# CompVis/zigma

Hardware: AMD Instinct MI355X
Metric: denoiser-forward latents/sec (BxL tokens/s), ZigMa d=640 L=32^2 (higher is better)
Workload: dtype bf16; 1 GPU; readme_text_b64: ZigMa(in_ch=3,img=32,E=640,depth=18,zigzagN8,has_text 77x768), B=64/GPU, bf16, one forward per step; global_batch=64, seq_len=1024, parallelism=batch-sharded x1

## Files before the change

zigma_amd/csrc/cross_attn.hip:

```cpp
#include "zigma_common.h"

namespace zigma {

typedef __bf16 bf16x8 __attribute__((ext_vector_type(8)));
typedef float f32x4 __attribute__((ext_vector_type(4)));

constexpr int kXaD = 64;
constexpr int kXaWaves = 4, kXaTok = 16;
constexpr int kXaKPitch = (kXaD + 8) * 2;


typedef float xa_f32x2 __attribute__((ext_vector_type(2)));
typedef __bf16 xa_bf16x2 __attribute__((ext_vector_type(2)));
__device__ __forceinline__ uint32_t pack_bf16(float lo, float hi) {
    return __builtin_bit_cast(uint32_t, __builtin_convertvector(xa_f32x2{lo, hi}, xa_bf16x2));
}

template <int NKB, bool MASK_ALL>
__global__ __launch_bounds__(64 * kXaWaves) void cross_attn_kernel(const zigma_xattn_params_t p, const int kXaTiles) {
    constexpr int KP = 16 * NKB;
    constexpr int KS = (KP + 31) / 32, KP2 = 32 * KS;
    constexpr int VPitch = (KP2 + 8) * 2;
    constexpr int OPitch = kXaKPitch;
    static_assert(VPitch >= OPitch, "the O tile reuses the P tile");
    __shared__ __attribute__((aligned(16))) unsigned char s_k[KP * kXaKPitch];
    __shared__ __attribute__((aligned(16))) unsigned char s_vt[kXaD * VPitch];
    __shared__ __attribute__((aligned(16))) unsigned char s_p[kXaWaves][kXaTok * VPitch];

    const int tid = threadIdx.x, lane = tid & 63;
    const int wave = __builtin_amdgcn_readfirstlane(tid >> 6);
    const int h = blockIdx.y, b = blockIdx.z, L = p.seqlen, NC = p.n_ctx;
    const int i16 = lane & 15, g = lane >> 4;
    const uint16_t *qb = reinterpret_cast<const uint16_t *>(p.q) + b * p.q_batch_stride + h * kXaD;
    const uint16_t *kb = reinterpret_cast<const uint16_t *>(p.k) + b * p.k_batch_stride + h * kXaD;
    const uint16_t *vb = reinterpret_cast<const uint16_t *>(p.v) + b * p.v_batch_stride + h * kXaD;
    uint16_t *ob = reinterpret_cast<uint16_t *>(p.out) + b * p.o_batch_stride + h * kXaD;

    for (int piece = tid; piece < KP * 8; piece += 64 * kXaWaves) {
        const int row = piece >> 3, pc = piece & 7;
        uint4 kv = make_uint4(0, 0, 0, 0);
        if (row < NC) kv = *reinterpret_cast<const uint4 *>(kb + row * p.k_row_stride + pc * 8);
        *reinterpret_cast<uint4 *>(s_k + row * kXaKPitch + pc * 16) = kv;
    }
    for (int unit = tid; unit < (KP2 / 8) * (kXaD / 2); unit += 64 * kXaWaves) {
        const int kg = unit / (kXaD / 2), dp = unit % (kXaD / 2);
        uint32_t w[8];
#pragma unroll
        for (int e = 0; e < 8; ++e) {
            const int key = kg * 8 + e;
            w[e] = key < NC ? *reinterpret_cast<const uint32_t *>(vb + key * p.v_row_stride + dp * 2) : 0u;
        }
        uint4 lo, hi;
        lo.x = (w[0] & 0xffffu) | (w[1] << 16); lo.y = (w[2] & 0xffffu) | (w[3] << 16);
        lo.z = (w[4] & 0xffffu) | (w[5] << 16); lo.w = (w[6] & 0xffffu) | (w[7] << 16);
        hi.x = (w[0] >> 16) | (w[1] & 0xffff0000u); hi.y = (w[2] >> 16) | (w[3] & 0xffff0000u);
        hi.z = (w[4] >> 16) | (w[5] & 0xffff0000u); hi.w = (w[6] >> 16) | (w[7] & 0xffff0000u);
        *reinterpret_cast<uint4 *>(s_vt + (2 * dp) * VPitch + kg * 16) = lo;
        *reinterpret_cast<uint4 *>(s_vt + (2 * dp + 1) * VPitch + kg * 16) = hi;
    }
    __syncthreads();

    const float sc = p.scale * kLog2e;
    unsigned char *pt = s_p[wave];
    const int tile0 = blockIdx.x * kXaTiles * kXaWaves + wave;
    auto load_q = [&](int t0, bf16x8 (&qa)[2]) {
        int tq = t0 + i16;
        tq = tq < L ? tq : L - 1;
        const uint16_t *qrow = qb + static_cast<int64_t>(tq) * p.q_row_stride;
#pragma unroll
        for (int ks = 0; ks < 2; ++ks) qa[ks] = __builtin_bit_cast(bf16x8, *reinterpret_cast<const uint4 *>(qrow + ks * 32 + g * 8));
    };
    bf16x8 qn[2];
    if (tile0 * kXaTok < L) load_q(tile0 * kXaTok, qn);
#pragma unroll 1
    for (int it = 0; it < kXaTiles; ++it) {
        const int t0 = (tile0 + it * kXaWaves) * kXaTok;
        if (t0 >= L) break;
        const bf16x8 qa[2] = {qn[0], qn[1]};
        if (it + 1 < kXaTiles && t0 + kXaWaves * kXaTok < L) load_q(t0 + kXaWaves * kXaTok, qn);
        f32x4 s[NKB];
#pragma unroll
        for (int ks = 0; ks < 2; ++ks) {
#pragma unroll
            for (int nb = 0; nb < NKB; ++nb) {
                const bf16x8 kf = __builtin_bit_cast(bf16x8, *reinterpret_cast<const uint4 *>(s_k + (nb * 16 + i16) * kXaKPitch + ks * 64 + g * 16));
                s[nb] = ks == 0 ? __builtin_amdgcn_mfma_f32_16x16x32_bf16(kf, qa[ks], f32x4{0.f, 0.f, 0.f, 0.f}, 0, 0, 0)
                                : __builtin_amdgcn_mfma_f32_16x16x32_bf16(kf, qa[ks], s[nb], 0, 0, 0);
            }
        }
        float m = -INFINITY;
#pragma unroll
        for (int nb = 0; nb < NKB; ++nb) {
#pragma unroll
            for (int r = 0; r < 4; ++r) {
                if (MASK_ALL || nb == NKB - 1) s[nb][r] = (nb * 16 + 4 * g + r < NC) ? s[nb][r] : -INFINITY;
                m = fmaxf(m, s[nb][r]);
            }
        }
        m = fmaxf(m, __shfl_xor(m, 16, 64));
        m = fmaxf(m, __shfl_xor(m, 32, 64));
        const float msc = -m * sc;
        float sum = 0.f;
#pragma unroll
        for (int nb = 0; nb < NKB; ++nb) {
            float e[4];
#pragma unroll
            for (int r = 0; r < 4; ++r) { e[r] = fast_exp2(__builtin_fmaf(s[nb][r], sc, msc)); sum += e[r]; }
            *reinterpret_cast<uint2 *>(pt + i16 * VPitch + (nb * 16 + 4 * g) * 2) = make_uint2(pack_bf16(e[0], e[1]), pack_bf16(e[2], e[3]));
        }
        if (KP2 > KP) *reinterpret_cast<uint2 *>(pt + i16 * VPitch + (KP + 4 * g) * 2) = make_uint2(0u, 0u);
        sum += __shfl_xor(sum, 16, 64);
        sum += __shfl_xor(sum, 32, 64);
        __builtin_amdgcn_fence(__ATOMIC_RELEASE, "wavefront");
        __builtin_amdgcn_wave_barrier();
        __builtin_amdgcn_fence(__ATOMIC_ACQUIRE, "wavefront");
        f32x4 o[4];
#pragma unroll
        for (int ks = 0; ks < KS; ++ks) {
            const bf16x8 pf = __builtin_bit_cast(bf16x8, *reinterpret_cast<const uint4 *>(pt + i16 * VPitch + ks * 64 + g * 16));
#pragma unroll
            for (int db = 0; db < 4; ++db) {
                const bf16x8 vf = __builtin_bit_cast(bf16x8, *reinterpret_cast<const uint4 *>(s_vt + (db * 16 + i16) * VPitch + ks * 64 + g * 16));
                o[db] = ks == 0 ? __builtin_amdgcn_mfma_f32_16x16x32_bf16(vf, pf, f32x4{0.f, 0.f, 0.f, 0.f}, 0, 0, 0)
                                : __builtin_amdgcn_mfma_f32_16x16x32_bf16(vf, pf, o[db], 0, 0, 0);
            }
        }
        __builtin_amdgcn_fence(__ATOMIC_RELEASE, "wavefront");
        __builtin_amdgcn_wave_barrier();
        const float inv = fast_rcp(sum);
#pragma unroll
        for (int db = 0; db < 4; ++db)
            *reinterpret_cast<uint2 *>(pt + i16 * OPitch + (db * 16 + 4 * g) * 2) =
                make_uint2(pack_bf16(o[db][0] * inv, o[db][1] * inv), pack_bf16(o[db][2] * inv, o[db][3] * inv));
        __builtin_amdgcn_fence(__ATOMIC_RELEASE, "wavefront");
        __builtin_amdgcn_wave_barrier();
        __builtin_amdgcn_fence(__ATOMIC_ACQUIRE, "wavefront");
#pragma unroll
        for (int q = 0; q < 2; ++q) {
            const int idx = lane + 64 * q, tok = idx >> 3, pc = idx & 7;
            if (t0 + tok < L)
                *reinterpret_cast<uint4 *>(ob + static_cast<int64_t>(t0 + tok) * p.o_row_stride + pc * 8) =
                    *reinterpret_cast<const uint4 *>(pt + tok * OPitch + pc * 16);
        }
        __builtin_amdgcn_fence(__ATOMIC_RELEASE, "wavefront");
        __builtin_amdgcn_wave_barrier();
    }
}

}

using namespace zigma;

extern "C" int zigma_cross_attn_fwd(const zigma_xattn_params_t *pp, void *stream_) {
    if (!pp) return ZIGMA_ERR_NULL;
    (void)hipGetLastError();
    const zigma_xattn_params_t &p = *pp;
    if (p.batch < 0 || p.seqlen < 0 || p.heads < 1 || p.n_ctx < 1) return ZIGMA_ERR_SHAPE;
    if (p.flags != 0) return ZIGMA_ERR_UNSUPPORTED;
    if (!(p.scale > 0.f) || !(p.scale < 3.0e38f)) return ZIGMA_ERR_UNSUPPORTED;
    if (p.batch == 0 || p.seqlen == 0) return ZIGMA_OK;
    if (!p.q || !p.k || !p.v || !p.out) return ZIGMA_ERR_NULL;
    if (p.dtype != ZIGMA_BF16) return ZIGMA_ERR_DTYPE;
    if (p.head_dim != kXaD || p.n_ctx > 128 || p.batch > 65535 || p.heads > 65535) return ZIGMA_ERR_SHAPE;
    auto mis = [](const void *q, int64_t rs, int64_t bs) { return reinterpret_cast<uintptr_t>(q) % 16 != 0 || rs % 8 != 0 || bs % 8 != 0; };
    if (mis(p.q, p.q_row_stride, p.q_batch_stride) || mis(p.k, p.k_row_stride, p.k_batch_stride) ||
        mis(p.v, p.v_row_stride, p.v_batch_stride) || mis(p.out, p.o_row_stride, p.o_batch_stride))
        return ZIGMA_ERR_STRIDE;
    const int tiles = p.seqlen >= 512 ? 8 : 4;
    const int tok_per_wg = kXaTok * kXaWaves * tiles;
    dim3 grid((p.seqlen + tok_per_wg - 1) / tok_per_wg, p.heads, p.batch), block(64 * kXaWaves);
    hipStream_t stream = static_cast<hipStream_t>(stream_);
    if (p.n_ctx <= 80) {
        if (p.n_ctx > 64) hipLaunchKernelGGL((cross_attn_kernel<5, false>), grid, block, 0, stream, p, tiles);
        else hipLaunchKernelGGL((cross_attn_kernel<5, true>), grid, block, 0, stream, p, tiles);
    } else {
        if (p.n_ctx > 112) hipLaunchKernelGGL((cross_attn_kernel<8, false>), grid, block, 0, stream, p, tiles);
        else hipLaunchKernelGGL((cross_attn_kernel<8, true>), grid, block, 0, stream, p, tiles);
    }
    set_last_kernel("cross_attn_mfma");
    return check_launch();
}
```

Measured before the change: 3.855 million tokens/s.

## Prefetch K/V into registers, ring-buffer Q loads, use 8 waves for long sequences

The cross-attention kernel now issues all global K and V loads into registers before any shared-memory stores, so the loads overlap instead of serialising load/store. Q tiles are prefetched through a configurable ring of register slots, and the refill is placed after the QK MFMAs, fenced by sched barriers. For seqlen >= 1024 the launch uses 8 waves per workgroup instead of 4, and waves_per_eu hints are added. Bounds branches become clamped loads and masks. The cost is higher register pressure and fewer workgroups along the sequence axis.

Measured after the change: 3.859 million tokens/s, median of 5. No clear change (+0.1%).

```diff
diff --git a/zigma_amd/csrc/cross_attn.hip b/zigma_amd/csrc/cross_attn.hip
--- a/zigma_amd/csrc/cross_attn.hip
+++ b/zigma_amd/csrc/cross_attn.hip
@@ -6,18 +6,29 @@
 typedef float f32x4 __attribute__((ext_vector_type(4)));
 
 constexpr int kXaD = 64;
-constexpr int kXaWaves = 4, kXaTok = 16;
+constexpr int kXaTok = 16;
+#ifndef ZIGMA_XA_WAVES8_MIN_L
+#define ZIGMA_XA_WAVES8_MIN_L 1024
+#endif
 constexpr int kXaKPitch = (kXaD + 8) * 2;
+#ifndef ZIGMA_XA_RING
+#define ZIGMA_XA_RING 1
+#endif
+#ifndef ZIGMA_XA_TILES
+#define ZIGMA_XA_TILES 8
+#endif
+constexpr int kXaRing = ZIGMA_XA_RING;
 
 
 typedef float xa_f32x2 __attribute__((ext_vector_type(2)));
 typedef __bf16 xa_bf16x2 __attribute__((ext_vector_type(2)));
+typedef uint32_t xa_u32x4 __attribute__((ext_vector_type(4)));
 __device__ __forceinline__ uint32_t pack_bf16(float lo, float hi) {
     return __builtin_bit_cast(uint32_t, __builtin_convertvector(xa_f32x2{lo, hi}, xa_bf16x2));
 }
 
-template <int NKB, bool MASK_ALL>
-__global__ __launch_bounds__(64 * kXaWaves) void cross_attn_kernel(const zigma_xattn_params_t p, const int kXaTiles) {
+template <int NKB, bool MASK_ALL, int kXaWaves>
+__global__ __launch_bounds__(64 * kXaWaves) __attribute__((amdgpu_waves_per_eu(NKB == 5 ? 4 : 3))) void cross_attn_kernel(const zigma_xattn_params_t p, const int kXaTiles) {
     constexpr int KP = 16 * NKB;
     constexpr int KS = (KP + 31) / 32, KP2 = 32 * KS;
     constexpr int VPitch = (KP2 + 8) * 2;
@@ -36,20 +47,66 @@
     const uint16_t *vb = reinterpret_cast<const uint16_t *>(p.v) + b * p.v_batch_stride + h * kXaD;
     uint16_t *ob = reinterpret_cast<uint16_t *>(p.out) + b * p.o_batch_stride + h * kXaD;
 
-    for (int piece = tid; piece < KP * 8; piece += 64 * kXaWaves) {
+    const int tile0 = blockIdx.x * kXaTiles * kXaWaves + wave;
+    const int rem = L - tile0 * kXaTok;
+    const int nt_all = (rem + kXaWaves * kXaTok - 1) / (kXaWaves * kXaTok);
+    const int nt = rem <= 0 ? 0 : (nt_all < kXaTiles ? nt_all : kXaTiles);
+    auto load_q = [&](int t0, xa_u32x4 (&qa)[2]) {
+        int tq = t0 + i16;
+        tq = tq < L ? tq : L - 1;
+        const uint16_t *qrow = qb + static_cast<int64_t>(tq) * p.q_row_stride;
+#pragma unroll
+        for (int ks = 0; ks < 2; ++ks) qa[ks] = *reinterpret_cast<const xa_u32x4 *>(qrow + ks * 32 + g * 8);
+    };
+    xa_u32x4 qr[kXaRing][2];
+#pragma unroll
+    for (int r = 0; r < kXaRing; ++r)
+        load_q(r < nt ? (tile0 + r * kXaWaves) * kXaTok : L, qr[r]);
+
+    constexpr int NT = 64 * kXaWaves, KPieces = KP * 8, VUnits = (KP2 / 8) * (kXaD / 2);
+    constexpr int KI = (KPieces + NT - 1) / NT, VI = (VUnits + NT - 1) / NT;
+    xa_u32x4 kreg[KI];
+    uint32_t vreg[VI][8];
+#pragma unroll
+    for (int i = 0; i < KI; ++i) {
+        int piece = tid + i * NT;
+        piece = piece < KPieces ? piece : KPieces - 1;
+        int row = piece >> 3;
+        row = row < NC ? row : NC - 1;
+        kreg[i] = *reinterpret_cast<const xa_u32x4 *>(kb + row * p.k_row_stride + (piece & 7) * 8);
+    }
+#pragma unroll
+    for (int i = 0; i < VI; ++i) {
+        int unit = tid + i * NT;
+        unit = unit < VUnits ? unit : VUnits - 1;
+        const int kg = unit / (kXaD / 2), dp = unit % (kXaD / 2);
+#pragma unroll
+        for (int e = 0; e < 8; ++e) {
+            int key = kg * 8 + e;
+            key = key < NC ? key : NC - 1;
+#ifdef ZIGMA_XA_PROBE_NO_V
+            vreg[i][e] = 0u;
+#else
+            vreg[i][e] = *reinterpret_cast<const uint32_t *>(vb + key * p.v_row_stride + dp * 2);
+#endif
+        }
+    }
+#pragma unroll
+    for (int i = 0; i < KI; ++i) {
+        int piece = tid + i * NT;
+        piece = piece < KPieces ? piece : KPieces - 1;
         const int row = piece >> 3, pc = piece & 7;
-        uint4 kv = make_uint4(0, 0, 0, 0);
-        if (row < NC) kv = *reinterpret_cast<const uint4 *>(kb + row * p.k_row_stride + pc * 8);
-        *reinterpret_cast<uint4 *>(s_k + row * kXaKPitch + pc * 16) = kv;
-    }
-    for (int unit = tid; unit < (KP2 / 8) * (kXaD / 2); unit += 64 * kXaWaves) {
+        const uint32_t keep = row < NC ? ~0u : 0u;
+        *reinterpret_cast<xa_u32x4 *>(s_k + row * kXaKPitch + pc * 16) = kreg[i] & keep;
+    }
+#pragma unroll
+    for (int i = 0; i < VI; ++i) {
+        int unit = tid + i * NT;
+        unit = unit < VUnits ? unit : VUnits - 1;
         const int kg = unit / (kXaD / 2), dp = unit % (kXaD / 2);
         uint32_t w[8];
 #pragma unroll
-        for (int e = 0; e < 8; ++e) {
-            const int key = kg * 8 + e;
-            w[e] = key < NC ? *reinterpret_cast<const uint32_t *>(vb + key * p.v_row_stride + dp * 2) : 0u;
-        }
+        for (int e = 0; e < 8; ++e) w[e] = kg * 8 + e < NC ? vreg[i][e] : 0u;
         uint4 lo, hi;
         lo.x = (w[0] & 0xffffu) | (w[1] << 16); lo.y = (w[2] & 0xffffu) | (w[3] << 16);
         lo.z = (w[4] & 0xffffu) | (w[5] << 16); lo.w = (w[6] & 0xffffu) | (w[7] << 16);
@@ -58,26 +115,14 @@
         *reinterpret_cast<uint4 *>(s_vt + (2 * dp) * VPitch + kg * 16) = lo;
         *reinterpret_cast<uint4 *>(s_vt + (2 * dp + 1) * VPitch + kg * 16) = hi;
     }
+    __builtin_amdgcn_s_waitcnt(0x0F70);
     __syncthreads();
 
     const float sc = p.scale * kLog2e;
     unsigned char *pt = s_p[wave];
-    const int tile0 = blockIdx.x * kXaTiles * kXaWaves + wave;
-    auto load_q = [&](int t0, bf16x8 (&qa)[2]) {
-        int tq = t0 + i16;
-        tq = tq < L ? tq : L - 1;
-        const uint16_t *qrow = qb + static_cast<int64_t>(tq) * p.q_row_stride;
-#pragma unroll
-        for (int ks = 0; ks < 2; ++ks) qa[ks] = __builtin_bit_cast(bf16x8, *reinterpret_cast<const uint4 *>(qrow + ks * 32 + g * 8));
-    };
-    bf16x8 qn[2];
-    if (tile0 * kXaTok < L) load_q(tile0 * kXaTok, qn);
-#pragma unroll 1
-    for (int it = 0; it < kXaTiles; ++it) {
+    auto do_tile = [&](const int it, xa_u32x4 (&slot)[2], const bool refill) __attribute__((always_inline)) {
         const int t0 = (tile0 + it * kXaWaves) * kXaTok;
-        if (t0 >= L) break;
-        const bf16x8 qa[2] = {qn[0], qn[1]};
-        if (it + 1 < kXaTiles && t0 + kXaWaves * kXaTok < L) load_q(t0 + kXaWaves * kXaTok, qn);
+        const bf16x8 qa[2] = {__builtin_bit_cast(bf16x8, slot[0]), __builtin_bit_cast(bf16x8, slot[1])};
         f32x4 s[NKB];
 #pragma unroll
         for (int ks = 0; ks < 2; ++ks) {
@@ -88,6 +133,11 @@
                                 : __builtin_amdgcn_mfma_f32_16x16x32_bf16(kf, qa[ks], s[nb], 0, 0, 0);
             }
         }
+        if (refill) {
+            __builtin_amdgcn_sched_barrier(0);
+            load_q(it + kXaRing < nt ? t0 + kXaRing * kXaWaves * kXaTok : L, slot);
+            __builtin_amdgcn_sched_barrier(0);
+        }
         float m = -INFINITY;
 #pragma unroll
         for (int nb = 0; nb < NKB; ++nb) {
@@ -137,13 +187,25 @@
         __builtin_amdgcn_fence(__ATOMIC_ACQUIRE, "wavefront");
 #pragma unroll
         for (int q = 0; q < 2; ++q) {
-            const int idx = lane + 64 * q, tok = idx >> 3, pc = idx & 7;
-            if (t0 + tok < L)
-                *reinterpret_cast<uint4 *>(ob + static_cast<int64_t>(t0 + tok) * p.o_row_stride + pc * 8) =
-                    *reinterpret_cast<const uint4 *>(pt + tok * OPitch + pc * 16);
-        }
-        __builtin_amdgcn_fence(__ATOMIC_RELEASE, "wavefront");
-        __builtin_amdgcn_wave_barrier();
+            const int idx = lane + 64 * q, pc = idx & 7;
+            int tok = idx >> 3;
+            tok = t0 + tok < L ? tok : L - 1 - t0;
+            *reinterpret_cast<uint4 *>(ob + static_cast<int64_t>(t0 + tok) * p.o_row_stride + pc * 8) =
+                *reinterpret_cast<const uint4 *>(pt + tok * OPitch + pc * 16);
+        }
+        __builtin_amdgcn_fence(__ATOMIC_RELEASE, "wavefront");
+        __builtin_amdgcn_wave_barrier();
+    };
+    int itb = 0;
+#pragma unroll 1
+    for (; itb + kXaRing <= nt; itb += kXaRing) {
+#pragma unroll
+        for (int r = 0; r < kXaRing; ++r) do_tile(itb + r, qr[r], true);
+    }
+#pragma unroll
+    for (int r = 0; r < kXaRing - 1; ++r) {
+        if (itb + r >= nt) break;
+        do_tile(itb + r, qr[r], false);
     }
 }
 
@@ -166,17 +228,20 @@
     if (mis(p.q, p.q_row_stride, p.q_batch_stride) || mis(p.k, p.k_row_stride, p.k_batch_stride) ||
         mis(p.v, p.v_row_stride, p.v_batch_stride) || mis(p.out, p.o_row_stride, p.o_batch_stride))
         return ZIGMA_ERR_STRIDE;
-    const int tiles = p.seqlen >= 512 ? 8 : 4;
-    const int tok_per_wg = kXaTok * kXaWaves * tiles;
-    dim3 grid((p.seqlen + tok_per_wg - 1) / tok_per_wg, p.heads, p.batch), block(64 * kXaWaves);
+    const int tiles = p.seqlen >= 512 ? ZIGMA_XA_TILES : 4;
+    const int waves = p.seqlen >= ZIGMA_XA_WAVES8_MIN_L ? 8 : 4;
+    const int tok_per_wg = kXaTok * waves * tiles;
+    dim3 grid((p.seqlen + tok_per_wg - 1) / tok_per_wg, p.heads, p.batch), block(64 * waves);
     hipStream_t stream = static_cast<hipStream_t>(stream_);
+#define ZIGMA_XA(NKB_, MASK_) \
+    if (waves == 8) hipLaunchKernelGGL((cross_attn_kernel<NKB_, MASK_, 8>), grid, block, 0, stream, p, tiles); \
+    else hipLaunchKernelGGL((cross_attn_kernel<NKB_, MASK_, 4>), grid, block, 0, stream, p, tiles);
     if (p.n_ctx <= 80) {
-        if (p.n_ctx > 64) hipLaunchKernelGGL((cross_attn_kernel<5, false>), grid, block, 0, stream, p, tiles);
-        else hipLaunchKernelGGL((cross_attn_kernel<5, true>), grid, block, 0, stream, p, tiles);
+        if (p.n_ctx > 64) { ZIGMA_XA(5, false) } else { ZIGMA_XA(5, true) }
     } else {
-        if (p.n_ctx > 112) hipLaunchKernelGGL((cross_attn_kernel<8, false>), grid, block, 0, stream, p, tiles);
-        else hipLaunchKernelGGL((cross_attn_kernel<8, true>), grid, block, 0, stream, p, tiles);
-    }
+        if (p.n_ctx > 112) { ZIGMA_XA(8, false) } else { ZIGMA_XA(8, true) }
+    }
+#undef ZIGMA_XA
     set_last_kernel("cross_attn_mfma");
     return check_launch();
 }
```
